# Jun-CEN/Open-World-Semantic-Segmentation

Measured on AMD Instinct MI355X. Metric: images/sec train-step, DeepLabV3+R101 768x768 bs=16; % HBM & MFMA roofline, higher is better.
Workload: dtype f16x2

## Files before the change

open-world-semantic-segmentation_amd/csrc/conv_choice.h:

```cpp
#pragma once
#include <cstdint>

#include "../../include/dmlnet_hip.h"

namespace conv_choice {

constexpr int CUS = 256;
constexpr int BK = 32;
constexpr int NTHREADS = 256;
constexpr int WS_MT = 9;
constexpr int WS_STAT_ROWS = 48;
constexpr int WS_NLD = 3;
constexpr int WB_THREADS = 512;
constexpr int WGW_TN = 128, WGW_TK = 256, WGW_NLD = 3;
constexpr int WG_MAX_JOBS = 12;

struct ConvSwitches {
    bool v1;
    int bm256, ws;
};

static inline int mul32(const int a, const int b) { return (int)((uint32_t)a * (uint32_t)b); }
static inline uintptr_t addr(const void* p) { return reinterpret_cast<uintptr_t>(p); }

static inline int64_t operand_bytes(const int B, const int Hi, const int Wi, const int ld, const int C, const int es) {
    return (((int64_t)mul32(B, Hi) * Wi - 1) * ld + C) * es;
}
static inline int blocks_for(const int64_t work_items, const int block, const int max_blocks = 256 * 8) {
    int64_t g = (work_items + block - 1) / block;
    if (g < 1) g = 1;
    if (g > max_blocks) g = max_blocks;
    return (int)g;
}

enum ConvFamily {
    CONV_REG = 0,
    CONV_RING,
    CONV_WS,
    CONV_X3
};

struct ConvChoice {
    int family;
    int elem_bytes;
    int mode;
    int bn, aligned;
    int bm, tmw, wpe;
    int mw, nw, pl, mt, epi;
    int nblk_m, nblk_n, tail_full, tail_q, nt_out;
    uint32_t x_bytes, w_bytes;
    uint32_t kx_bytes, kw_bytes;
    int grid, block;
    int stat_rows;
};

static inline int conv_m(const DmlConvDesc& d) { return mul32(mul32(d.B, d.Ho), d.Wo); }
static inline int conv_ktot(const DmlConvDesc& d) { return mul32(mul32(d.R, d.S), d.C); }
static inline int conv_f32_split(const DmlConvDesc& d) { return d.dtype == DML_F32 ? d.f32_split : 0; }
static inline bool conv_has_planes(const DmlConvDesc& d) { return conv_f32_split(d) == 2 && d.x_planes && d.w_planes; }
static inline bool conv_has_tail(const DmlConvDesc& d) { return d.tail_ws && d.tail_counters && d.tail_ws_elems > 0 && d.tail_counters_len > 0; }
static inline int conv_pad_x(const DmlConvDesc& d) { return d.pad_w_set ? d.pad_w : d.pad; }

static inline int64_t conv_x_bytes(const DmlConvDesc& d, const int es) { return operand_bytes(d.B, d.Hi, d.Wi, d.ldx, d.C, es); }
static inline int64_t conv_w_bytes(const DmlConvDesc& d, const int es) { return (int64_t)d.N * conv_ktot(d) * es; }

static inline bool conv_dma_eligible(const DmlConvDesc& d, const ConvSwitches& sw, const int64_t xb, const int64_t wb) {
    return !sw.v1 && (d.C % BK) == 0 && d.R * d.S <= 32 && d.N > 32 && xb < (1ll << 31) && wb < (1ll << 31);
}

static inline bool conv_ws_eligible(const DmlConvDesc& d, const ConvSwitches& sw, const int64_t xb, const int64_t wb) {
    if ((!sw.ws && d.ws_min_tiles <= 0) || !d.w_tiled || (d.C % BK) != 0 || d.R * d.S > 32 || (d.N % 128) != 0) return false;
    if (xb >= (1ll << 31) || wb >= (1ll << 31)) return false;
    if (d.ws_min_tiles <= 0 && d.R * d.S * d.C < 1024) return false;
    const int bn = (d.N % 256) == 0 ? 256 : 128, bm = (d.N % 256) == 0 ? 144 : 288;
    const int64_t ntiles = ((int64_t)conv_m(d) + bm - 1) / bm * (d.N / bn);
    return ntiles >= (d.ws_min_tiles > 0 ? d.ws_min_tiles : 192);
}
static inline bool ws_planes_short(const DmlConvDesc& d, const int mode) {
    return mode == 0 && (d.N % 256) == 0 && ((conv_m(d) + 143) / 144) * (d.N / 256) * 2 <= 256;
}
static inline int ws_planes_stat_rows(const DmlConvDesc& d, const int mode) {
    if (mode != 0) return 48;
    return (d.N == 64 || ws_planes_short(d, mode)) ? 48 : 144;
}
static inline bool conv_ws_planes_eligible(const DmlConvDesc& d, const int mode) {
    if (mode == 0 && d.accum) return false;
    if (!conv_has_planes(d) || !d.x_unscale || !d.w_unscale) return false;
    if (d.x_plane_stride >= (1ll << 30) || d.w_plane_stride >= (1ll << 30)) return false;
    if ((d.C % BK) != 0 || d.R * d.S > 32 || (d.N % 64) != 0) return false;
    if (mode == 1 && conv_ktot(d) < 2 * BK) return false;
    const bool post = d.post_scale != nullptr;
    if ((d.ldy & 3) != 0 || (post && d.post_res != nullptr && (d.post_ldres & 3) != 0) ||
        ((addr(d.y) | addr(d.bias) | (post ? addr(d.post_res) | addr(d.post_scale) | addr(d.post_shift) | addr(d.post_mean) : 0)) & 15) != 0)
        return false;
    return conv_x_bytes(d, 2) + (uint32_t)(d.x_plane_stride * 2) < (1ll << 31) && conv_w_bytes(d, 2) + (uint32_t)(d.w_plane_stride * 2) < (1ll << 31);
}

static inline int tail_split(const DmlConvDesc& d, const int ntiles, const int tile_rows, const int max_full, int* full_out) {
// ... 99 lines not shown
    *c = ConvChoice{};
    c->stat_rows = DML_STAT_ROWS;
    if (!dp) return DML_EINVAL;
    const DmlConvDesc& d = *dp;
    const bool planes_ok = d.dtype == DML_F32 && conv_ws_planes_eligible(d, d.mode);
    bool ws_ok = false;
    if (d.dtype == DML_BF16) {
        const int64_t xb = conv_x_bytes(d, 2), wb = conv_w_bytes(d, 2);
        ws_ok = conv_dma_eligible(d, sw, xb, wb) && conv_ws_eligible(d, sw, xb, wb);
    }
    if (planes_ok) c->stat_rows = ws_planes_stat_rows(d, d.mode);
    else if (ws_ok) c->stat_rows = WS_STAT_ROWS;

    if (!d.x || !d.w || !d.y) return DML_EINVAL;
    if (d.dtype != DML_F32 && d.dtype != DML_BF16) return DML_EINVAL;
    const int vec = d.dtype == DML_BF16 ? 8 : 4;
    if (d.C % vec || d.ldx % vec) return DML_EALIGN;
    if (d.mode != 0 && d.mode != 1) return DML_EINVAL;
    if (d.mode == 1 && d.stride != 1 && d.stride != 2) return DML_EUNSUPPORTED;
    if (d.B <= 0 || d.Ho <= 0 || d.Wo <= 0 || d.N <= 0 || d.R <= 0 || d.S <= 0) return DML_EINVAL;
    if ((int64_t)d.B * d.Ho * d.Wo >= (1ll << 31)) return DML_EINVAL;
    if (d.stats && d.bias) return DML_EINVAL;
    const int f32_split = conv_f32_split(d);
    if (f32_split < 0 || f32_split > 2) return DML_EINVAL;
    if (conv_has_planes(d)) {
        if (!d.x_unscale || !d.w_unscale || d.x_plane_stride <= 0 || d.w_plane_stride <= 0 ||
            d.x_plane_stride >= (1ll << 30) || d.w_plane_stride >= (1ll << 30))
            return DML_EINVAL;
        if ((addr(d.x_planes) & 15) || (addr(d.w_planes) & 15) || (d.x_plane_stride & 7) || (d.w_plane_stride & 7)) return DML_EALIGN;
    }
    if (d.w_tiled && (d.dtype != DML_BF16 || d.C % BK || d.N % 64)) return DML_EUNSUPPORTED;
    if (d.acc32) {
        if (d.mode != 1 || d.dtype != DML_BF16 || d.y_f32 || d.accum || d.res_dz || d.bnr_partials) return DML_EINVAL;
        if (d.N % 8 || d.ldy % 8 || d.acc32_ld % 4 || (addr(d.y) & 15) || (addr(d.acc32) & 15) || d.N <= 32) return DML_EALIGN;
    }
    if (d.res_dz) {
        if (d.mode != 1 || d.y_f32 || d.accum || !d.res_mask) return DML_EINVAL;
        if (d.dtype == DML_BF16) {
            if (d.N % 8 || d.ldy % 8 || d.res_ld % 8 || (addr(d.y) & 15) || (addr(d.res_dz) & 15) || d.N <= 32) return DML_EALIGN;
            if ((d.N & 63) == 0 && (addr(d.res_mask) & 7)) return DML_EALIGN;
        } else if (d.N % 64 || d.res_ld % 4 || ((addr(d.res_dz) | addr(d.res_mask)) & 15)) {
            return DML_EALIGN;
        }
    }
    if (conv_has_tail(d) && (addr(d.tail_ws) & 15)) return DML_EALIGN;
    if (d.post_scale) {
        if (d.mode != 0 || !d.post_shift || !d.post_mean || d.stats || d.bias || d.accum || d.y_f32) return DML_EINVAL;
        if (d.post_res && (d.post_ldres % vec || (addr(d.post_res) & 15))) return DML_EALIGN;
    }
    if (d.bnr_partials) {
        if (d.mode != 1 || d.y_f32 || !d.bnr_y || !d.bnr_mean || !d.bnr_invstd || (d.bnr_relu && !d.bnr_mask)) return DML_EINVAL;
        if (d.dtype == DML_BF16) {
            if (d.N % 8 || d.ldy % 8 || d.bnr_ldy % 8 || (addr(d.y) & 15) || (addr(d.bnr_y) & 15) || (addr(d.bnr_partials) & 15) || d.N <= 32)
                return DML_EUNSUPPORTED;
            if (d.bnr_relu && (d.N & 63) == 0 && (addr(d.bnr_mask) & 7)) return DML_EALIGN;
        } else {
            if (d.N % 64 || d.bnr_ldy % 4) return DML_EUNSUPPORTED;
            if (((addr(d.bnr_y) | addr(d.bnr_partials) | addr(d.bnr_mean) | addr(d.bnr_invstd) | (d.bnr_relu ? addr(d.bnr_mask) : 0)) & 15) != 0)
                return DML_EALIGN;
        }
    }
    if (d.bnr_partials && d.bnr_inc != 0 && (!d.accum || d.dtype != DML_F32 || d.res_dz)) return DML_EUNSUPPORTED;
    if (d.sub_grid) {
        if (d.mode != 1 || d.stride != 1 || d.dil != 1 || d.Hi != d.Ho || d.Wi != d.Wo || (unsigned)d.sub_y > 1u || (unsigned)d.sub_x > 1u ||
            d.dtype != DML_F32)
            return DML_EINVAL;
        if ((int64_t)4 * d.B * d.Ho * d.Wo * (int64_t)d.ldy * 4 >= (1ll << 31)) return DML_EUNSUPPORTED;
    }
    const bool own_geometry = d.sub_grid || conv_pad_x(d) != d.pad;
    if (own_geometry && (d.dtype == DML_BF16 || d.acc32)) return DML_EUNSUPPORTED;
    if (d.acc32) return conv_choose_kernel(d, sw, 2, 2, ws_ok, false, c);
    if (d.dtype == DML_BF16) return conv_choose_kernel(d, sw, 2, d.mode, ws_ok, false, c);
    if ((d.bnr_partials || d.res_dz || own_geometry) && !planes_ok) return DML_EUNSUPPORTED;
    if (d.f32_split == 2 && d.x_planes && d.x == d.x_planes && !planes_ok) return DML_EUNSUPPORTED;
    return conv_choose_kernel(d, sw, 4, d.mode, false, planes_ok, c);
}

enum WgradFamily {
    WGRAD_BIG = 0,
    WGRAD_WS,
    WGRAD_H2,
    WGRAD_N64,
    WGRAD_X3,
    WGRAD_PLAIN
};

struct ReduceLaunch {
    int grid_x, grid_y, block, splits, slab_stride, fold_only;
};

struct WgradChoice {
    int family;
    int lin;
    int elem_bytes;
    bool planes;
    bool use_ws;
    int tiles, cm;
    int nblk_n, nblk_k, splitk, slab_tiles;
    int grid, block;
    uint32_t x_bytes, dy_bytes;
    int nitems;
    int64_t nrs;
    int nreduce;
    ReduceLaunch reduce[2];
};

static inline int64_t wgrad_m(const DmlWgradDesc& d) { return (int64_t)d.B * d.Ho * d.Wo; }
static inline int wgrad_ktot(const DmlWgradDesc& d) { return mul32(mul32(d.R, d.S), d.C); }
static inline int64_t wgrad_x_bytes(const DmlWgradDesc& d, const int es) { return operand_bytes(d.B, d.Hi, d.Wi, d.ldx, d.C, es); }
static inline int64_t wgrad_dy_bytes(const DmlWgradDesc& d, const int es) { return ((wgrad_m(d) - 1) * d.ldy + d.N) * es; }

static inline bool wgrad_big_eligible(const DmlWgradDesc* d, const bool group) {
    if (!d) return false;
    const int64_t M = wgrad_m(*d), Ktot = (int64_t)d->R * d->S * d->C, tiles = (M + BK - 1) / BK;
    if (group) {
        if (!d->x || !d->dy || !d->dw) return false;
        if (d->C % 8 || d->ldx % 8 || d->N % 8 || d->ldy % 8) return false;
        if ((d->Cm > 0 ? d->Cm : d->C) > d->C) return false;
        if ((int64_t)d->N * Ktot < 65536) return false;
    }
    return d->dtype == DML_BF16 && d->N % 256 == 0 && (d->N / 256) * ((Ktot + 255) / 256) >= 4 && tiles >= 16 &&
           wgrad_x_bytes(*d, 2) < (1ll << 31) && wgrad_dy_bytes(*d, 2) < (1ll << 31) && (int64_t)(d->B + 1) * d->Hi * d->Wi < (1 << 24) &&
           M < (1 << 24) && d->ldx < (1 << 22) && d->ldy < (1 << 22);
}

template <class Score>
static inline int pick_splits(const int tiles, const int min_steps, const int64_t plane, const int64_t ws_elems, Score score) {
    int smax = tiles / min_steps;
    if (smax > 256) smax = 256;
    if ((int64_t)smax * plane > ws_elems) smax = (int)(ws_elems / plane);
    if (smax < 1) smax = 1;
    double best = -1e30;
    int sk = 1;
    for (int c = 1; c <= smax; ++c) {
        const int slab = (tiles + c - 1) / c;
        const int real = (tiles + slab - 1) / slab;
        const double s = score(slab, real);
        if (s > best + 1e-9) { best = s; sk = real; }
    }
    return sk;
}
static inline int flat_splits(const int base, const int tiles, const bool use_ws) {
    int splitk = use_ws ? (512 + base - 1) / base : (1024 + base - 1) / base;
    if (use_ws && tiles / 48 > splitk) splitk = tiles / 48;
    const int cap = (tiles + 7) / 8;
    if (splitk > cap) splitk = cap;
    if (splitk < 1) splitk = 1;
    return splitk;
}
static inline int finish_splits(int sk, const int tiles, const bool use_ws, const int64_t plane, const int64_t ws_elems, int* slab_tiles) {
    if (use_ws && (int64_t)sk * plane > ws_elems) sk = (int)(ws_elems / plane);
    if (use_ws && sk < 1) return 0;
    if (sk > tiles) sk = tiles > 0 ? tiles : 1;
    *slab_tiles = (tiles + sk - 1) / sk;
    return (tiles + *slab_tiles - 1) / *slab_tiles;
}

static inline int wgrad_choose(const DmlWgradDesc* dp, WgradChoice* c) {
    *c = WgradChoice{};
    if (!dp || !dp->x || !dp->dy || !dp->dw) return DML_EINVAL;
    const DmlWgradDesc& d = *dp;
    if (d.dtype != DML_F32 && d.dtype != DML_BF16) return DML_EINVAL;
    const int vec = d.dtype == DML_BF16 ? 8 : 4;
    if (d.C % vec || d.ldx % vec || d.N % vec || d.ldy % vec) return DML_EALIGN;
    if (wgrad_m(d) >= (1ll << 31)) return DML_EINVAL;
    const int M = (int)wgrad_m(d), Ktot = wgrad_ktot(d), N = d.N;
    if (d.dtype == DML_F32 && d.f32_split == 2 && d.x_planes && d.dy_planes) {
        if (!d.x_unscale || !d.dy_unscale || d.x_plane_stride <= 0 || d.dy_plane_stride <= 0) return DML_EINVAL;
        if ((addr(d.x_planes) & 15) || (addr(d.dy_planes) & 15) || (d.x_plane_stride & 7) || (d.dy_plane_stride & 7)) return DML_EALIGN;
        c->planes = d.C % 8 == 0 && d.N % 8 == 0 && d.ldx % 8 == 0 && d.ldy % 8 == 0 &&
                    wgrad_x_bytes(d, 2) + d.x_plane_stride * 2 < 0x7fffffffll && wgrad_dy_bytes(d, 2) + d.dy_plane_stride * 2 < 0x7fffffffll;
    }
    if (!c->planes && ((d.x_planes && d.x == d.x_planes) || (d.dy_planes && d.dy == d.dy_planes))) return DML_EUNSUPPORTED;
    const int tiles = c->tiles = (M + BK - 1) / BK;
    const int cm = c->cm = d.Cm > 0 ? d.Cm : d.C;
    if (cm > d.C) return DML_EINVAL;
    if (cm != d.C && !d.ws) return DML_EINVAL;
    const int64_t plane = (int64_t)N * Ktot;
    const bool use_ws = c->use_ws = d.ws != nullptr;
    c->lin = (d.R == 1 && d.S == 1 && d.stride == 1 && d.pad == 0) ? 1 : 0;
    c->nrs = (int64_t)N * d.R * d.S;
    c->block = NTHREADS;
    int sk = d.splitk, rblock = 256, rmax = 256 * 8;
    if (use_ws && wgrad_big_eligible(dp, false)) {
        c->family = WGRAD_BIG;
        c->nblk_n = N / 256;
        c->nblk_k = (Ktot + 255) / 256;
        const int base = c->nblk_n * c->nblk_k;
        if (sk <= 0)
            sk = pick_splits(tiles, 8, plane, d.ws_elems, [&](const int, const int real) {
                const int blocks = base * real;
                const int rnd = base < 6 ? 128 : 256;
                return (double)blocks / (double)(((blocks + rnd - 1) / rnd) * rnd);
            });
        c->block = WB_THREADS;
        c->x_bytes = (uint32_t)wgrad_x_bytes(d, 2);
        c->dy_bytes = (uint32_t)wgrad_dy_bytes(d, 2);
    } else if (c->planes && use_ws && N % WGW_TN == 0 && tiles >= 16 && (addr(d.ws) & 15) == 0) {
        c->family = WGRAD_WS;
        c->nblk_n = N / WGW_TN;
        c->nblk_k = (Ktot + WGW_TK - 1) / WGW_TK;
        const int base = c->nblk_n * c->nblk_k;
        if (sk <= 0)
            sk = pick_splits(tiles, 16, plane, d.ws_elems, [&](const int slab, const int real) {
                const int items = base * real;
                return -((double)((items + 255) / 256) * (slab * 1.45 + 8.0) + (double)real * (double)plane * 8.0 / 4.0e6);
            });
        c->block = (4 + WGW_NLD) * 64;
        c->x_bytes = (uint32_t)wgrad_x_bytes(d, 2);
        c->dy_bytes = (uint32_t)wgrad_dy_bytes(d, 2);
        rblock = 64;
        rmax = 256 * 8 * (256 / rblock);
    } else {
        const bool n64 = d.dtype == DML_BF16 && N <= 64 && d.R * d.S > 1;
        c->nblk_n = n64 ? 1 : (N + 127) / 128;
        c->nblk_k = n64 ? (Ktot + 255) / 256 : (Ktot + 127) / 128;
        if (sk <= 0) sk = flat_splits(c->nblk_n * c->nblk_k, tiles, use_ws);
        const int64_t x3_xb = wgrad_x_bytes(d, 4), x3_yb = wgrad_dy_bytes(d, 4);
        if (c->planes) {
            c->family = WGRAD_H2;
            c->x_bytes = (uint32_t)wgrad_x_bytes(d, 2);
            c->dy_bytes = (uint32_t)wgrad_dy_bytes(d, 2);
        } else if (n64) {
            c->family = WGRAD_N64;
        } else if (d.dtype == DML_F32 && d.f32_split && x3_xb < (int64_t)0x7fffffff && x3_yb < (int64_t)0x7fffffff) {
            c->family = WGRAD_X3;
            c->x_bytes = (uint32_t)x3_xb;
            c->dy_bytes = (uint32_t)x3_yb;
        } else {
            c->family = WGRAD_PLAIN;
            c->elem_bytes = d.dtype == DML_BF16 ? 2 : 4;
        }
    }
    sk = c->splitk = finish_splits(sk, tiles, use_ws, plane, d.ws_elems, &c->slab_tiles);
    if (sk < 1) return DML_EINVAL;
    c->grid = c->nblk_n * c->nblk_k * sk;
    if (c->family == WGRAD_WS) {
        c->nitems = c->grid;
        c->grid = c->nitems < 256 ? c->nitems : 256;
    }
    if (use_ws) {
        const int gx = blocks_for(c->nrs * cm, rblock, rmax);
        const int ychunks = (c->family != WGRAD_BIG && c->family != WGRAD_WS && c->nrs * cm < 65536 && sk > 64) ? (sk + 15) / 16 : 1;
        if (ychunks > 1) {
            c->nreduce = 2;
            c->reduce[0] = ReduceLaunch{gx, ychunks, rblock, sk, 1, 1};
            c->reduce[1] = ReduceLaunch{gx, 1, rblock, ychunks, 16, 0};
        } else {
            c->nreduce = 1;
            c->reduce[0] = ReduceLaunch{gx, 1, rblock, sk, 1, 0};
        }
    }
    return 0;
}

struct WgradGroupChoice {
    int n;
    int nblk_n[WG_MAX_JOBS], nblk_k[WG_MAX_JOBS], splitk[WG_MAX_JOBS], slab_tiles[WG_MAX_JOBS], cm[WG_MAX_JOBS];
    uint32_t x_bytes[WG_MAX_JOBS], dy_bytes[WG_MAX_JOBS];
    int64_t ws_off[WG_MAX_JOBS], nrs[WG_MAX_JOBS];
    int start[WG_MAX_JOBS + 1];
    int grid, block;
    int rgrid_x, rgrid_y, rblock;
};

static inline int wgrad_group_choose(const DmlWgradDesc* const* descs, const int n, const void* ws, const int64_t ws_elems, WgradGroupChoice* g) {
    *g = WgradGroupChoice{};
    if (!descs || n <= 0 || n > WG_MAX_JOBS || !ws) return DML_EINVAL;
    int base[WG_MAX_JOBS], tiles[WG_MAX_JOBS], sk[WG_MAX_JOBS];
    int64_t plane[WG_MAX_JOBS];
    double work = 0.0;
    int tbase = 0;
    for (int j = 0; j < n; ++j) {
        const DmlWgradDesc* d = descs[j];
        if (!wgrad_big_eligible(d, true)) return DML_EUNSUPPORTED;
        const int Ktot = wgrad_ktot(*d);
        g->nblk_n[j] = d->N / 256;
        g->nblk_k[j] = (Ktot + 255) / 256;
// ... 54 lines not shown
```

open-world-semantic-segmentation_amd/csrc/conv_device.h:

```cpp
#pragma once
#include "common.h"
#include "conv_choice.h"

namespace conv_device {

struct ConvArgs {
    const void* x;
    const void* w;
    void* y;
    const float* bias;
    float* stats;
    int B, Hi, Wi, C, ldx;
    int Ho, Wo, N, ldy;
    int R, S, stride, dil, pad;
    int M, Ktot;
    int y_f32, accum;
    int nblk_n, nblk_m;
    FastDiv div_wo, div_howo, div_c;
    float* unused0_;
    uint32_t x_bytes, w_bytes;
    int w_tiled;
    int ws_min_tiles;
    const void* x_planes;
    const void* w_planes;
    const float* x_unscale;
    const float* w_unscale;
    uint32_t x_plane_bytes, w_plane_bytes;
    const void* bnr_y;
    const uint8_t* bnr_mask;
    const float* bnr_mean;
    const float* bnr_invstd;
    float* bnr_partials;
    float* bnr_gmax;
    int bnr_ldy, bnr_relu;
    const float* post_scale;
    const float* post_shift;
    const float* post_mean;
    const void* post_res;
    int post_ldres, post_relu;
    float* tail_ws;
    int* tail_cnt;
    int tail_full, tail_q;
    int64_t tail_ws_elems_;
    int tail_cnt_len_;
    const void* res_dz;
    const uint8_t* res_mask;
    int res_ld;
    const float* acc32;
    int acc32_ld;
    int f32_split;
    int nt_out;
    int unused1_;
    int pad_x;
    int sub_grid, sub_y, sub_x;
    int bnr_inc;
};

__attribute__((visibility("hidden"))) void launch_conv_ws(const conv_choice::ConvChoice& c, const ConvArgs& a, hipStream_t st);
__attribute__((visibility("hidden"))) void launch_conv_ws_dgrad_planes(const conv_choice::ConvChoice& c, const ConvArgs& a, hipStream_t st);

}

namespace {

using namespace conv_device;
namespace cc = conv_choice;

constexpr int BK = 32;
constexpr int NTHREADS = 256;
constexpr int WS_MT = 9;
constexpr int WS_STAT_ROWS = 48;
constexpr int WS_NST = 6, WS_D = 2;
constexpr int WS_PLANES_NLD = 3;

typedef __bf16 mfma_bf16x8 __attribute__((ext_vector_type(8)));
typedef _Float16 mfma_f16x8 __attribute__((ext_vector_type(8)));
typedef unsigned int u32x4_ws __attribute__((ext_vector_type(4)));
typedef __attribute__((address_space(3))) void* lds_ptr_t;
template <int N> __device__ __forceinline__ void wait_vmcnt() { asm volatile("s_waitcnt vmcnt(%0)" ::"n"(N) : "memory"); }

__device__ __forceinline__ uint32_t ws_out_row(const ConvArgs& a, const uint32_t m) {
    if (!a.sub_grid) return m;
    if (m >= (uint32_t)a.M) return 4u * (uint32_t)a.M;
    const uint32_t b = fdiv(m, a.div_howo);
    const uint32_t rem = m - b * (uint32_t)(a.Ho * a.Wo);
    const uint32_t y2 = fdiv(rem, a.div_wo);
    const uint32_t x2 = rem - y2 * (uint32_t)a.Wo;
    return ((b * 2u * (uint32_t)a.Ho + 2u * y2 + (uint32_t)a.sub_y) * 2u * (uint32_t)a.Wo) + 2u * x2 + (uint32_t)a.sub_x;
}
__device__ __forceinline__ uint32_t ws_out_rows(const ConvArgs& a) { return a.sub_grid ? 4u * (uint32_t)a.M : (uint32_t)a.M; }

constexpr int WGRAD_DEPTH = 2;

__device__ __forceinline__ int xcd_remap(int bid, int nwg) {
    const int q = nwg >> 3, r = nwg & 7, xcd = bid & 7, slot = bid >> 3;
    const int base = xcd < r ? xcd * (q + 1) : r * (q + 1) + (xcd - r) * q;
    return base + slot;
}

template <typename T> __device__ __forceinline__ int swz_chunk(int row, int chunk);
template <> __device__ __forceinline__ int swz_chunk<bf16_t>(int row, int chunk) {
    return chunk ^ ((0x78 >> (((row >> 2) & 3) * 2)) & 3);
}
template <> __device__ __forceinline__ int swz_chunk<float>(int row, int chunk) { return chunk ^ (row & 7); }

template <int NT> __device__ __forceinline__ int frag_chan(int i, int g) {
    return NT == 4 ? (i >> 1) * 32 + g * 8 + (i & 1) * 4 : g * (4 * NT) + i * 4;
}
template <int NT> __device__ __forceinline__ int b_row(int i, int rho) { return frag_chan<NT>(i, rho >> 2) + (rho & 3); }
template <int NT> __device__ __forceinline__ int b_rho(int row) {
    return NT == 4 ? ((row >> 3) & 3) * 4 + (row & 3) : ((row / (4 * NT)) & 3) * 4 + (row & 3);
}

template <int CTRL> __device__ __forceinline__ float dpp_mov(float v) {
    return __int_as_float(__builtin_amdgcn_update_dpp(0, __float_as_int(v), CTRL, 0xF, 0xF, true));
}
__device__ __forceinline__ float row16_sum(float v) {
    v += dpp_mov<0xB1>(v);
    v += dpp_mov<0x4E>(v);
    v += dpp_mov<0x141>(v);
    v += dpp_mov<0x140>(v);
    return v;
}

typedef unsigned int u32x4_st __attribute__((ext_vector_type(4)));
typedef float f32x4_st __attribute__((ext_vector_type(4)));
__device__ __forceinline__ void st16(void* p, uint32_t a, uint32_t b, uint32_t c, uint32_t d, const bool nt) {
    const u32x4_st v = {a, b, c, d};
    if (nt) asm volatile("global_store_dwordx4 %0, %1, off nt" ::"v"(p), "v"(v) : "memory");
    else *reinterpret_cast<u32x4_st*>(p) = v;
}
__device__ __forceinline__ void st16f(float* p, float a, float b, float c, float d, const bool nt) {
    const f32x4_st v = {a, b, c, d};
    if (nt) asm volatile("global_store_dwordx4 %0, %1, off nt" ::"v"(p), "v"(v) : "memory");
    else *reinterpret_cast<f32x4_st*>(p) = v;
}

template <typename T, int NT, int MT, int MODE, bool WIDE_MASK = true, bool STATS_ONLY = false>
__device__ __forceinline__ void conv_epilogue(f32x4 (&acc)[NT][MT], const ConvArgs& a, const int mw0, const int nw0,
                                              const int lr, const int lq) {
    constexpr int TM = MT * 16;
    constexpr int CL = NT * 4;
    auto ch = [&](int c) { return nw0 + frag_chan<NT>(c >> 2, lq) + (c & 3); };

    if (a.stats != nullptr) {
        const int cnt = min(TM, max(0, a.M - mw0));
        if (cnt > 0) {
            const float inv = 1.0f / (float)cnt;
            const int grp = mw0 / TM;
            float* sg = a.stats + (int64_t)grp * a.N * 2;
            const bool pair_ok = (a.N & 1) == 0;
            const bool gather = pair_ok && nw0 + NT * 16 <= a.N;
            float S[NT][4], Q[NT][4];
#pragma unroll
            for (int i = 0; i < NT; ++i) {
                float s[4] = {0.f, 0.f, 0.f, 0.f};
#pragma unroll
                for (int j = 0; j < MT; ++j) {
                    const bool v = (mw0 + j * 16 + lr) < a.M;
#pragma unroll
                    for (int q = 0; q < 4; ++q) s[q] += v ? acc[i][j][q] : 0.f;
                }
#pragma unroll
                for (int q = 0; q < 4; ++q) s[q] = row16_sum(s[q]);
                float m2[4] = {0.f, 0.f, 0.f, 0.f};
#pragma unroll
                for (int j = 0; j < MT; ++j) {
                    const bool v = (mw0 + j * 16 + lr) < a.M;
#pragma unroll
                    for (int q = 0; q < 4; ++q) {
                        const float dlt = acc[i][j][q] - s[q] * inv;
                        m2[q] += v ? dlt * dlt : 0.f;
                    }
// ... 284 lines not shown
```

open-world-semantic-segmentation_amd/csrc/conv_igemm.hip:

```cpp
#include "conv_device.h"
#include <cstdlib>

namespace {

template <typename T, int BN, bool ALIGNED, int MODE>
__global__ __launch_bounds__(NTHREADS) __attribute__((amdgpu_waves_per_eu(3))) void conv_igemm_kernel(const ConvArgs a) {
    constexpr int BM = 128;
    constexpr int VEC = Elem<T>::VEC;
    constexpr int KV = BK / VEC;
    constexpr int RPP = NTHREADS / KV;
    constexpr int A_LD = BM / RPP;
    constexpr int B_LD = (BN + RPP - 1) / RPP;
    constexpr int TM = 64, TN = BN / 2;
    constexpr int MT = TM / 16, NT = TN / 16;

    __shared__ __attribute__((aligned(256))) T smem[2 * (BM + BN) * BK];
    auto As = [&](int buf) -> T* { return smem + buf * (BM + BN) * BK; };
    auto Bs = [&](int buf) -> T* { return smem + buf * (BM + BN) * BK + BM * BK; };

    const int tid = threadIdx.x, lane = tid & 63, wave = tid >> 6;
    const int wm = wave >> 1, wn = wave & 1;
    const int tile = xcd_remap(blockIdx.x, gridDim.x);
    const int blk_m = tile / a.nblk_n, blk_n = tile - blk_m * a.nblk_n;
    const int m0 = blk_m * BM, n0 = blk_n * BN;
// ... 548 lines not shown
        if (LA > 2 && kt + 2 < KT) wait_vmcnt<(LA > 2 ? 2 : 0) * NI>();
        else if (LA > 1 && kt + 1 < KT) wait_vmcnt<(LA > 1 ? 1 : 0) * NI>();
        else wait_vmcnt<0>();
        __builtin_amdgcn_s_barrier();
        if (kt + LA < KT) issue(kbeg + kt + LA, (kt + LA) % NST);
        const T* as = smem + (kt % NST) * STAGE + (wm * TM) * BK;
        const T* bs = smem + (kt % NST) * STAGE + BM * BK + (wn * TN) * BK;
        mfma_bf16x8 bf[NT], af[MT];
#pragma unroll
        for (int i = 0; i < NT; ++i)
            bf[i] = *reinterpret_cast<const mfma_bf16x8*>(bs + b_row<NT>(i, lr) * BK + swz_chunk<T>(lr, lq) * 8);
#pragma unroll
        for (int j = 0; j < MT; ++j) {
            const int row = j * 16 + lr;
            af[j] = *reinterpret_cast<const mfma_bf16x8*>(as + row * BK + swz_chunk<T>(row, lq) * 8);
        }
#pragma unroll
        for (int i = 0; i < NT; ++i)
#pragma unroll
            for (int j = 0; j < MT; ++j)
                acc[i][j] = __builtin_amdgcn_mfma_f32_16x16x32_bf16(bf[i], af[j], acc[i][j], 0, 0, 0);
    }
#pragma unroll
    for (int i = 0; i < NT; ++i)
#pragma unroll
        for (int j = 0; j < MT; ++j) asm volatile("" : "+v"(acc[i][j]));
    if (kparts > 1) {
        const int rt = tile - a.tail_full;
        typedef unsigned int u32x4_t __attribute__((ext_vector_type(4)));
        const __amdgpu_buffer_rsrc_t rs_ws = __builtin_amdgcn_make_buffer_rsrc(
            a.tail_ws + (int64_t)rt * kparts * (BM * BN), 0, kparts * BM * BN * 4, 0x00020000);
#pragma unroll
        for (int i = 0; i < NT; ++i)
#pragma unroll
            for (int j = 0; j < MT; ++j)
                __builtin_amdgcn_raw_buffer_store_b128(__builtin_bit_cast(u32x4_t, acc[i][j]), rs_ws,
                                                       (kpart * BM * BN + ((i * MT + j) * NTH + tid) * 4) * 4, 0, 16);
        asm volatile("s_waitcnt vmcnt(0)" ::: "memory");
        __syncthreads();
        int* flag = reinterpret_cast<int*>(smem);
        if (tid == 0) {
            const int ticket = __hip_atomic_fetch_add(a.tail_cnt + rt, 1, __ATOMIC_RELAXED, __HIP_MEMORY_SCOPE_AGENT);
            if (ticket == kparts - 1)
                __hip_atomic_store(a.tail_cnt + rt, 0, __ATOMIC_RELAXED, __HIP_MEMORY_SCOPE_AGENT);
            *flag = ticket;
        }
        __syncthreads();
        if (*flag != kparts - 1) return;
#pragma unroll
        for (int i = 0; i < NT; ++i)
#pragma unroll
            for (int j = 0; j < MT; ++j) acc[i][j] = (f32x4){0.f, 0.f, 0.f, 0.f};
        for (int p = 0; p < kparts; ++p) {
#pragma unroll
            for (int i = 0; i < NT; ++i)
#pragma unroll
                for (int j = 0; j < MT; ++j) {
                    const u32x4_t v = __builtin_amdgcn_raw_buffer_load_b128(
                        rs_ws, (p * BM * BN + ((i * MT + j) * NTH + tid) * 4) * 4, 0, 16);
                    acc[i][j] += __builtin_bit_cast(f32x4, v);
                }
        }
    }
    if constexpr (MT == 4) {
        conv_epilogue<T, NT, MT, MODE>(acc, a, m0 + wm * TM, n0 + wn * TN, lr, lq);
    } else {
#pragma unroll
        for (int h = 0; h < MT / 4; ++h) {
            f32x4 sub[NT][4];
#pragma unroll
            for (int i = 0; i < NT; ++i)
#pragma unroll
                for (int j = 0; j < 4; ++j) sub[i][j] = acc[i][h * 4 + j];
            conv_epilogue<T, NT, 4, MODE, false>(sub, a, m0 + wm * TM + h * 64, n0 + wn * TN, lr, lq);
        }
    }
}

static const conv_choice::ConvSwitches& conv_switches() {
    static const conv_choice::ConvSwitches s = {getenv("DML_CONV_V1") != nullptr, getenv("DML_CONV_BM256") ? atoi(getenv("DML_CONV_BM256")) : 1,
                                                getenv("DML_CONV_WS") ? atoi(getenv("DML_CONV_WS")) : 0};
    return s;
}

struct WgradArgs {
    const void* x;
    const void* dy;
    float* dw;
    int B, Hi, Wi, C, ldx;
    int Ho, Wo, N, ldy;
    int R, S, stride, dil, pad;
    int M, Ktot;
    int nblk_n, nblk_k;
    int slab_tiles;
    float* ws;
    FastDiv div_wo, div_howo, div_c;
    const void* x_planes;
    const void* dy_planes;
    const float* x_unscale;
    const float* dy_unscale;
    uint32_t x_plane_bytes, dy_plane_bytes;
};

template <typename T> struct WgLds;
template <> struct WgLds<float> { static constexpr int PITCH = 128 + 16; };
template <> struct WgLds<bf16_t> { static constexpr int PITCH = 128 + 8; };

__device__ __forceinline__ bf16x4 lds_tr16_b64(const bf16_t* p) {
    typedef short v4i16 __attribute__((ext_vector_type(4)));
    return __builtin_amdgcn_ds_read_tr16_b64_v4i16((v4i16 __attribute__((address_space(3)))*)(p));
}

template <typename T>
__global__ __launch_bounds__(NTHREADS) void conv_wgrad_kernel(const WgradArgs a) {
    constexpr int TILE = 128;
    constexpr int VEC = Elem<T>::VEC;
    constexpr int CV = TILE / VEC;
    constexpr int RPP = NTHREADS / CV;
    constexpr int LD = BK / RPP;
    constexpr int PITCH = WgLds<T>::PITCH;
    constexpr int MT = 4, NT = 4;

    __shared__ __attribute__((aligned(16))) T smem[2 * 2 * BK * PITCH];
    auto Ys = [&](int buf) -> T* { return smem + buf * 2 * BK * PITCH; };
    auto Xs = [&](int buf) -> T* { return smem + buf * 2 * BK * PITCH + BK * PITCH; };

    const int tid = threadIdx.x, lane = tid & 63, wave = tid >> 6;
    const int wn = wave >> 1, wk = wave & 1;
    const int ntile = a.nblk_n * a.nblk_k;
    const int logical = xcd_remap(blockIdx.x, gridDim.x);
    const int split = logical / ntile, tile_id = logical - split * ntile;
    const int blk_n = tile_id % a.nblk_n, blk_k = tile_id / a.nblk_n;
    const int n0 = blk_n * TILE, kc0 = blk_k * TILE;

    const T* __restrict__ X = static_cast<const T*>(a.x);
    const T* __restrict__ DY = static_cast<const T*>(a.dy);

    const int vcol = tid % CV, prow = tid / CV;
    const int kc = kc0 + vcol * VEC;
    const bool kc_ok = kc < a.Ktot;
    const uint32_t tap = fdiv((uint32_t)(kc_ok ? kc : 0), a.div_c);
    const int xc = (kc_ok ? kc : 0) - (int)tap * a.C;
    const int tr = (int)tap / a.S, ts = (int)tap - tr * a.S;
    const int dyo = tr * a.dil - a.pad, dxo = ts * a.dil - a.pad;
    const int yn = n0 + vcol * VEC;
    const bool yn_ok = yn < a.N;

    const int tile_beg = split * a.slab_tiles;
    const int tiles_total = (a.M + BK - 1) / BK;
    const int tile_end = min(tiles_total, tile_beg + a.slab_tiles);

    const bool lin1x1 = a.R == 1 && a.S == 1 && a.stride == 1 && a.pad == 0;
    uint4 y_reg[LD], x_reg[LD];
    auto load_tiles = [&](int t) {
#pragma unroll
        for (int j = 0; j < LD; ++j) {
            const int m = t * BK + prow + j * RPP;
            uint4 yv = make_uint4(0, 0, 0, 0), xv = make_uint4(0, 0, 0, 0);
            if (m < a.M) {
                if (yn_ok) yv = *reinterpret_cast<const uint4*>(DY + (int64_t)m * a.ldy + yn);
                if (kc_ok && lin1x1) {
                    xv = *reinterpret_cast<const uint4*>(X + (int64_t)m * a.ldx + xc);
                } else if (kc_ok) {
                    const uint32_t b = fdiv((uint32_t)m, a.div_howo);
                    const uint32_t rem = (uint32_t)m - b * (uint32_t)(a.Ho * a.Wo);
                    const uint32_t yo = fdiv(rem, a.div_wo);
                    const uint32_t xo = rem - yo * (uint32_t)a.Wo;
                    const int ys = (int)yo * a.stride + dyo, xs = (int)xo * a.stride + dxo;
                    if ((unsigned)ys < (unsigned)a.Hi && (unsigned)xs < (unsigned)a.Wi)
                        xv = *reinterpret_cast<const uint4*>(
                            X + ((int64_t)((int)b * a.Hi + ys) * a.Wi + xs) * a.ldx + xc);
                }
            }
            y_reg[j] = yv;
            x_reg[j] = xv;
        }
    };
    auto store_tiles = [&](int buf) {
#pragma unroll
        for (int j = 0; j < LD; ++j) {
            const int row = prow + j * RPP;
            int off;
            if constexpr (sizeof(T) == 2) {
                const int prow_ = (row & 0x13) | (((row >> 3) & 1) << 2) | (((row >> 2) & 1) << 3);
                off = (vcol >> 1) * 528 + prow_ * 16 + (vcol & 1) * 8;
            } else {
                off = row * PITCH + vcol * VEC;
            }
            *reinterpret_cast<uint4*>(Ys(buf) + off) = y_reg[j];
            *reinterpret_cast<uint4*>(Xs(buf) + off) = x_reg[j];
        }
    };

    f32x4 acc[NT][MT];
// ... 1053 lines not shown

template <typename T, int MODE>
void launch_conv(const cc::ConvChoice& c, const ConvArgs& a, hipStream_t st) {
    const dim3 grid(c.grid), block(c.block);
    switch (c.family) {
    case cc::CONV_RING:
        if constexpr (sizeof(T) == 2) {
            if (c.bm == 256)
                hipLaunchKernelGGL((conv_igemm_dma_kernel<128, MODE, 3, 2, 256, 128>), grid, block, 0, st, a, c.kx_bytes, c.kw_bytes);
            else if (c.bn == 128)
                hipLaunchKernelGGL((conv_igemm_dma_kernel<128, MODE, 3>), grid, block, 0, st, a, c.kx_bytes, c.kw_bytes);
            else
                hipLaunchKernelGGL((conv_igemm_dma_kernel<64, MODE, 3>), grid, block, 0, st, a, c.kx_bytes, c.kw_bytes);
        }
        break;
    case cc::CONV_X3:
        if constexpr (sizeof(T) == 4 && MODE != 2) {
            if (c.bn == 128) hipLaunchKernelGGL((conv_igemm_x3_kernel<128, MODE>), grid, block, 0, st, a);
            else hipLaunchKernelGGL((conv_igemm_x3_kernel<64, MODE>), grid, block, 0, st, a);
        }
        break;
    default:
        if constexpr (MODE != 2) {
            if (c.aligned) {
                if (c.bn == 128) hipLaunchKernelGGL((conv_igemm_kernel<T, 128, true, MODE>), grid, block, 0, st, a);
                else if (c.bn == 64) hipLaunchKernelGGL((conv_igemm_kernel<T, 64, true, MODE>), grid, block, 0, st, a);
                else hipLaunchKernelGGL((conv_igemm_kernel<T, 32, true, MODE>), grid, block, 0, st, a);
            } else {
                if (c.bn == 128) hipLaunchKernelGGL((conv_igemm_kernel<T, 128, false, MODE>), grid, block, 0, st, a);
                else if (c.bn == 64) hipLaunchKernelGGL((conv_igemm_kernel<T, 64, false, MODE>), grid, block, 0, st, a);
                else hipLaunchKernelGGL((conv_igemm_kernel<T, 32, false, MODE>), grid, block, 0, st, a);
            }
        }
        break;
    }
}

static void fill_wgrad_args(WgradArgs& a, const DmlWgradDesc* d, const bool planes) {
    a.x = d->x; a.dy = d->dy; a.dw = d->dw;
    a.B = d->B; a.Hi = d->Hi; a.Wi = d->Wi; a.C = d->C; a.ldx = d->ldx;
    a.Ho = d->Ho; a.Wo = d->Wo; a.N = d->N; a.ldy = d->ldy;
    a.R = d->R; a.S = d->S; a.stride = d->stride; a.dil = d->dil; a.pad = d->pad;
    a.M = d->B * d->Ho * d->Wo;
    a.Ktot = d->R * d->S * d->C;
    a.div_wo = make_fastdiv((uint32_t)d->Wo);
    a.div_howo = make_fastdiv((uint32_t)(d->Ho * d->Wo));
    a.div_c = make_fastdiv((uint32_t)d->C);
    a.x_planes = planes ? d->x_planes : nullptr; a.dy_planes = planes ? d->dy_planes : nullptr;
    a.x_unscale = planes ? d->x_unscale : nullptr; a.dy_unscale = planes ? d->dy_unscale : nullptr;
    a.x_plane_bytes = planes ? (uint32_t)(d->x_plane_stride * 2) : 0u;
    a.dy_plane_bytes = planes ? (uint32_t)(d->dy_plane_stride * 2) : 0u;
}

}

extern "C" int dml_conv_stat_rows(const DmlConvDesc* d) {
    cc::ConvChoice c;
    cc::conv_choose(d, conv_switches(), &c);
    return c.stat_rows;
}

extern "C" int dml_conv_igemm(const DmlConvDesc* d, void* stream) {
    cc::ConvChoice c;
    const int rc = cc::conv_choose(d, conv_switches(), &c);
    if (rc) return rc;
    const ConvArgs a = conv_args(d, c);
    hipStream_t st = static_cast<hipStream_t>(stream);
    if (c.family == cc::CONV_WS) {
        launch_conv_ws(c, a, st);
    } else if (c.elem_bytes == 2) {
        if (c.mode == 2) launch_conv<bf16_t, 2>(c, a, st);
        else if (c.mode == 1) launch_conv<bf16_t, 1>(c, a, st);
        else launch_conv<bf16_t, 0>(c, a, st);
    } else {
        if (c.mode == 1) launch_conv<float, 1>(c, a, st);
        else launch_conv<float, 0>(c, a, st);
    }
    DML_LAUNCH_CHECK();
    return 0;
}

extern "C" int dml_conv_wgrad(const DmlWgradDesc* d, void* stream) {
    cc::WgradChoice c;
    const int rc = cc::wgrad_choose(d, &c);
    if (rc) return rc;
    WgradArgs a;
    fill_wgrad_args(a, d, c.planes);
    a.nblk_n = c.nblk_n; a.nblk_k = c.nblk_k; a.slab_tiles = c.slab_tiles;
    a.ws = c.use_ws ? d->ws : nullptr;
    hipStream_t st = static_cast<hipStream_t>(stream);
    const dim3 grid(c.grid), block(c.block);
    switch (c.family) {
    case cc::WGRAD_BIG:
        hipLaunchKernelGGL(conv_wgrad_big_kernel<WGRAD_DEPTH>, grid, block, 0, st, a, c.x_bytes, c.dy_bytes);
        break;
    case cc::WGRAD_WS:
        if (c.lin) hipLaunchKernelGGL(conv_wgrad_ws_kernel<true>, grid, block, 0, st, a, c.x_bytes, c.dy_bytes, c.nitems);
        else hipLaunchKernelGGL(conv_wgrad_ws_kernel<false>, grid, block, 0, st, a, c.x_bytes, c.dy_bytes, c.nitems);
        break;
    case cc::WGRAD_H2:
        if (c.lin) hipLaunchKernelGGL(conv_wgrad_h2_kernel<true>, grid, block, 0, st, a, c.x_bytes, c.dy_bytes);
        else hipLaunchKernelGGL(conv_wgrad_h2_kernel<false>, grid, block, 0, st, a, c.x_bytes, c.dy_bytes);
        break;
    case cc::WGRAD_N64:
        hipLaunchKernelGGL(conv_wgrad_n64_kernel, grid, block, 0, st, a);
        break;
    case cc::WGRAD_X3:
        if (c.lin) hipLaunchKernelGGL(conv_wgrad_x3_kernel<true>, grid, block, 0, st, a, c.x_bytes, c.dy_bytes);
        else hipLaunchKernelGGL(conv_wgrad_x3_kernel<false>, grid, block, 0, st, a, c.x_bytes, c.dy_bytes);
        break;
    default:
        if (c.elem_bytes == 2) hipLaunchKernelGGL(conv_wgrad_kernel<bf16_t>, grid, block, 0, st, a);
        else hipLaunchKernelGGL(conv_wgrad_kernel<float>, grid, block, 0, st, a);
        break;
    }
    for (int i = 0; i < c.nreduce; ++i) {
        const cc::ReduceLaunch& r = c.reduce[i];
        hipLaunchKernelGGL(wgrad_reduce_kernel, dim3(r.grid_x, r.grid_y), dim3(r.block), 0, st, d->ws, d->dw, r.splits, c.nrs, c.cm, d->C,
                           r.slab_stride, r.fold_only);
    }
    DML_LAUNCH_CHECK();
    return 0;
}

extern "C" int dml_conv_wgrad_group_eligible(const DmlWgradDesc* d) { return cc::wgrad_big_eligible(d, true) ? 1 : 0; }

extern "C" int dml_conv_wgrad_group(const DmlWgradDesc* const* descs, int n, float* ws, int64_t ws_elems, void* stream) {
    cc::WgradGroupChoice c;
    const int rc = cc::wgrad_group_choose(descs, n, ws, ws_elems, &c);
    if (rc) return rc;
    WgradGroup g;
    ReduceGroup r;
    g.njobs = r.njobs = n;
    g.start[0] = 0;
    for (int j = 0; j < n; ++j) {
        const DmlWgradDesc* d = descs[j];
        WgradArgs& a = g.job[j];
        fill_wgrad_args(a, d, false);
        a.nblk_n = c.nblk_n[j]; a.nblk_k = c.nblk_k[j]; a.slab_tiles = c.slab_tiles[j];
        a.ws = ws + c.ws_off[j];
        g.xb[j] = c.x_bytes[j]; g.yb[j] = c.dy_bytes[j];
        g.start[j + 1] = c.start[j + 1];
        r.ws[j] = a.ws; r.dw[j] = d->dw; r.splits[j] = c.splitk[j]; r.Cm[j] = c.cm[j]; r.Cp[j] = d->C;
        r.NRS[j] = c.nrs[j];
    }
    hipStream_t st = static_cast<hipStream_t>(stream);
    hipLaunchKernelGGL(conv_wgrad_group_kernel<WGRAD_DEPTH>, dim3(c.grid), dim3(c.block), 0, st, g);
    hipLaunchKernelGGL(wgrad_reduce_group_kernel, dim3(c.rgrid_x, c.rgrid_y), dim3(c.rblock), 0, st, r);
    DML_LAUNCH_CHECK();
    return 0;
}
```

Baseline: 213.4.

## Add tap-reuse wgrad kernel for 64-channel 3x3 stride-1 convolutions

Adds a dedicated weight-gradient kernel for 3x3, pad-1, stride-1 convolutions with 64 input and output channels. It loads one input patch per row tile into LDS and reuses it for all nine taps, with a 3-stage async DMA pipeline over split f16 planes. The kernel computes hi/lo cross products with MFMA and writes split-K partials to the workspace for the existing reduce. It is on by default through an env switch and only applies to that narrow shape, so its effect on the whole train step depends on how many such layers DeepLabV3+ R101 has.

```diff
diff --git a/open-world-semantic-segmentation_amd/csrc/conv_choice.h b/open-world-semantic-segmentation_amd/csrc/conv_choice.h
--- a/open-world-semantic-segmentation_amd/csrc/conv_choice.h
+++ b/open-world-semantic-segmentation_amd/csrc/conv_choice.h
@@ -14,6 +14,8 @@
 constexpr int WB_THREADS = 512;
 constexpr int WGW_TN = 128, WGW_TK = 256, WGW_NLD = 3;
 constexpr int WG_MAX_JOBS = 12;
+constexpr int WGT_CH = 64;
+constexpr int WGT_MIN_STEPS = 8;
 
 struct ConvSwitches {
     bool v1;
@@ -279,7 +281,12 @@
     WGRAD_H2,
     WGRAD_N64,
     WGRAD_X3,
-    WGRAD_PLAIN
+    WGRAD_PLAIN,
+    WGRAD_TAP
+};
+
+struct WgradSwitches {
+    bool tap = false;
 };
 
 struct ReduceLaunch {
@@ -353,7 +360,12 @@
     return (tiles + *slab_tiles - 1) / *slab_tiles;
 }
 
-static inline int wgrad_choose(const DmlWgradDesc* dp, WgradChoice* c) {
+static inline bool wgrad_tap_eligible(const DmlWgradDesc& d, const bool planes, const bool use_ws) {
+    return planes && use_ws && (addr(d.ws) & 15) == 0 && d.R == 3 && d.S == 3 && d.stride == 1 && d.dil == 1 && d.pad == 1 &&
+           d.Hi == d.Ho && d.Wi == d.Wo && d.N == WGT_CH && d.C == WGT_CH && d.Wo % BK == 0;
+}
+
+static inline int wgrad_choose(const DmlWgradDesc* dp, WgradChoice* c, const WgradSwitches& sw = WgradSwitches{}) {
     *c = WgradChoice{};
     if (!dp || !dp->x || !dp->dy || !dp->dw) return DML_EINVAL;
     const DmlWgradDesc& d = *dp;
@@ -391,6 +403,14 @@
                 return (double)blocks / (double)(((blocks + rnd - 1) / rnd) * rnd);
             });
         c->block = WB_THREADS;
+        c->x_bytes = (uint32_t)wgrad_x_bytes(d, 2);
+        c->dy_bytes = (uint32_t)wgrad_dy_bytes(d, 2);
+    } else if (sw.tap && wgrad_tap_eligible(d, c->planes, use_ws)) {
+        c->family = WGRAD_TAP;
+        c->nblk_n = c->nblk_k = 1;
+        if (sk <= 0)
+            sk = pick_splits(tiles, WGT_MIN_STEPS, plane, d.ws_elems, [&](const int, const int real) { return (double)real / (double)CUS; });
+        if (sk > CUS) sk = CUS;
         c->x_bytes = (uint32_t)wgrad_x_bytes(d, 2);
         c->dy_bytes = (uint32_t)wgrad_dy_bytes(d, 2);
     } else if (c->planes && use_ws && N % WGW_TN == 0 && tiles >= 16 && (addr(d.ws) & 15) == 0) {
diff --git a/open-world-semantic-segmentation_amd/csrc/conv_device.h b/open-world-semantic-segmentation_amd/csrc/conv_device.h
--- a/open-world-semantic-segmentation_amd/csrc/conv_device.h
+++ b/open-world-semantic-segmentation_amd/csrc/conv_device.h
@@ -56,8 +56,28 @@
     int bnr_inc;
 };
 
+struct WgradArgs {
+    const void* x;
+    const void* dy;
+    float* dw;
+    int B, Hi, Wi, C, ldx;
+    int Ho, Wo, N, ldy;
+    int R, S, stride, dil, pad;
+    int M, Ktot;
+    int nblk_n, nblk_k;
+    int slab_tiles;
+    float* ws;
+    FastDiv div_wo, div_howo, div_c;
+    const void* x_planes;
+    const void* dy_planes;
+    const float* x_unscale;
+    const float* dy_unscale;
+    uint32_t x_plane_bytes, dy_plane_bytes;
+};
+
 __attribute__((visibility("hidden"))) void launch_conv_ws(const conv_choice::ConvChoice& c, const ConvArgs& a, hipStream_t st);
 __attribute__((visibility("hidden"))) void launch_conv_ws_dgrad_planes(const conv_choice::ConvChoice& c, const ConvArgs& a, hipStream_t st);
+__attribute__((visibility("hidden"))) void launch_conv_wgrad_tap(const conv_choice::WgradChoice& c, const WgradArgs& a, hipStream_t st);
 
 }
 
@@ -89,6 +109,11 @@
     return ((b * 2u * (uint32_t)a.Ho + 2u * y2 + (uint32_t)a.sub_y) * 2u * (uint32_t)a.Wo) + 2u * x2 + (uint32_t)a.sub_x;
 }
 __device__ __forceinline__ uint32_t ws_out_rows(const ConvArgs& a) { return a.sub_grid ? 4u * (uint32_t)a.M : (uint32_t)a.M; }
+
+__device__ __forceinline__ bf16x4 lds_tr16_b64(const bf16_t* p) {
+    typedef short v4i16 __attribute__((ext_vector_type(4)));
+    return __builtin_amdgcn_ds_read_tr16_b64_v4i16((v4i16 __attribute__((address_space(3)))*)(p));
+}
 
 constexpr int WGRAD_DEPTH = 2;
 
diff --git a/open-world-semantic-segmentation_amd/csrc/conv_igemm.hip b/open-world-semantic-segmentation_amd/csrc/conv_igemm.hip
--- a/open-world-semantic-segmentation_amd/csrc/conv_igemm.hip
+++ b/open-world-semantic-segmentation_amd/csrc/conv_igemm.hip
@@ -654,34 +654,14 @@
                                                 getenv("DML_CONV_WS") ? atoi(getenv("DML_CONV_WS")) : 0};
     return s;
 }
-
-struct WgradArgs {
-    const void* x;
-    const void* dy;
-    float* dw;
-    int B, Hi, Wi, C, ldx;
-    int Ho, Wo, N, ldy;
-    int R, S, stride, dil, pad;
-    int M, Ktot;
-    int nblk_n, nblk_k;
-    int slab_tiles;
-    float* ws;
-    FastDiv div_wo, div_howo, div_c;
-    const void* x_planes;
-    const void* dy_planes;
-    const float* x_unscale;
-    const float* dy_unscale;
-    uint32_t x_plane_bytes, dy_plane_bytes;
-};
+static const conv_choice::WgradSwitches& wgrad_switches() {
+    static const conv_choice::WgradSwitches s = {getenv("DML_WGRAD_TAP") ? atoi(getenv("DML_WGRAD_TAP")) != 0 : true};
+    return s;
+}
 
 template <typename T> struct WgLds;
 template <> struct WgLds<float> { static constexpr int PITCH = 128 + 16; };
 template <> struct WgLds<bf16_t> { static constexpr int PITCH = 128 + 8; };
-
-__device__ __forceinline__ bf16x4 lds_tr16_b64(const bf16_t* p) {
-    typedef short v4i16 __attribute__((ext_vector_type(4)));
-    return __builtin_amdgcn_ds_read_tr16_b64_v4i16((v4i16 __attribute__((address_space(3)))*)(p));
-}
 
 template <typename T>
 __global__ __launch_bounds__(NTHREADS) void conv_wgrad_kernel(const WgradArgs a) {
@@ -1901,7 +1881,7 @@
 
 extern "C" int dml_conv_wgrad(const DmlWgradDesc* d, void* stream) {
     cc::WgradChoice c;
-    const int rc = cc::wgrad_choose(d, &c);
+    const int rc = cc::wgrad_choose(d, &c, wgrad_switches());
     if (rc) return rc;
     WgradArgs a;
     fill_wgrad_args(a, d, c.planes);
@@ -1924,6 +1904,9 @@
     case cc::WGRAD_N64:
         hipLaunchKernelGGL(conv_wgrad_n64_kernel, grid, block, 0, st, a);
         break;
+    case cc::WGRAD_TAP:
+        launch_conv_wgrad_tap(c, a, st);
+        break;
     case cc::WGRAD_X3:
         if (c.lin) hipLaunchKernelGGL(conv_wgrad_x3_kernel<true>, grid, block, 0, st, a, c.x_bytes, c.dy_bytes);
         else hipLaunchKernelGGL(conv_wgrad_x3_kernel<false>, grid, block, 0, st, a, c.x_bytes, c.dy_bytes);
diff --git a/open-world-semantic-segmentation_amd/csrc/conv_wgrad_tap.hip b/open-world-semantic-segmentation_amd/csrc/conv_wgrad_tap.hip
--- /dev/null
+++ b/open-world-semantic-segmentation_amd/csrc/conv_wgrad_tap.hip
@@ -0,0 +1,143 @@
+#include "conv_device.h"
+
+namespace {
+
+constexpr int WGT_NST = 3;
+constexpr int WGT_PITCH = 32;
+constexpr int WGT_ROWPX = BK + 2, WGT_SLOTS = 3 * WGT_ROWPX;
+constexpr int WGT_YSUB = BK * WGT_PITCH;
+constexpr int WGT_XSUB = 4 * 1024;
+constexpr int WGT_YPL = 4 * WGT_YSUB, WGT_XPL = 4 * WGT_XSUB;
+constexpr int WGT_SB = 2 * WGT_YPL + 2 * WGT_XPL;
+constexpr int WGT_NI = 10;
+constexpr int WGT_KF = 18;
+static_assert(cc::WGT_CH == 64 && cc::BK == BK && 2 * WGT_KF * 16 == 9 * cc::WGT_CH, "conv_choice.h describes this kernel");
+static_assert((2 * WGT_ROWPX + 2 + BK) <= WGT_SLOTS && WGT_SLOTS * WGT_PITCH <= WGT_XSUB, "every tap's window lies inside the patch");
+
+__device__ __forceinline__ mfma_f16x8 wgt_frag(const char* p) {
+    const bf16x4 lo = lds_tr16_b64(reinterpret_cast<const bf16_t*>(p));
+    const bf16x4 hi = lds_tr16_b64(reinterpret_cast<const bf16_t*>(p + 16 * WGT_PITCH));
+    const bf16x8 v = {lo[0], lo[1], lo[2], lo[3], hi[0], hi[1], hi[2], hi[3]};
+    return __builtin_bit_cast(mfma_f16x8, v);
+}
+
+__device__ __forceinline__ constexpr int wgt_x_off(const int f) {
+    return 2 * WGT_YPL + (f & 3) * WGT_XSUB + (((f >> 2) / 3) * WGT_ROWPX + ((f >> 2) % 3)) * WGT_PITCH;
+}
+
+template <int WK>
+__device__ __forceinline__ void wgt_body(const WgradArgs& a, const u32x4_ws rs_x, const u32x4_ws rs_y, char* smem,
+                                         const int wave, const int lane, const int split, const int tile_beg, const int KT) {
+    constexpr uint32_t OOB = 0x80000000u;
+    const int wn = wave >> 1;
+    const int lr = lane & 15, lq = lane >> 4;
+
+    const int vec_b = (wave * 2 + (lane & 1)) * 16;
+    int x_dy[4], x_dx[4], x_off[4];
+#pragma unroll
+    for (int q = 0; q < 4; ++q) {
+        const int slot = q * 32 + (lane >> 1);
+        const int row = slot / WGT_ROWPX, col = slot - row * WGT_ROWPX;
+        x_dy[q] = slot < WGT_SLOTS ? row - 1 : -(1 << 20);
+        x_dx[q] = col - 1;
+        x_off[q] = ((row - 1) * a.Wi + (col - 1)) * (a.ldx * 2) + vec_b;
+    }
+    const int y_off = (lane >> 1) * (a.ldy * 2) + vec_b;
+    const uint32_t lds0 = (uint32_t)(uintptr_t)smem;
+    auto issue = [&](const int kt) {
+        const uint32_t sb = lds0 + (uint32_t)((kt % WGT_NST) * WGT_SB);
+        const uint32_t m0 = (uint32_t)(tile_beg + kt) * BK;
+        const uint32_t b = fdiv(m0, a.div_howo);
+        const uint32_t rem = m0 - b * (uint32_t)(a.Ho * a.Wo);
+        const int yo = (int)fdiv(rem, a.div_wo);
+        const int xo = (int)rem - yo * a.Wo;
+        const int base = (((int)b * a.Hi + yo) * a.Wi + xo) * (a.ldx * 2);
+#pragma unroll
+        for (int q = 0; q < 4; ++q) {
+            const bool ok = (unsigned)(yo + x_dy[q]) < (unsigned)a.Hi && (unsigned)(xo + x_dx[q]) < (unsigned)a.Wi;
+            const uint32_t voff = ok ? (uint32_t)(base + x_off[q]) : OOB;
+            const uint32_t dst = sb + (uint32_t)(2 * WGT_YPL + wave * WGT_XSUB + q * 1024);
+            ws_dma16(rs_x, dst, voff, 0u);
+            ws_dma16(rs_x, dst + WGT_XPL, voff, a.x_plane_bytes);
+        }
+        const uint32_t yv = m0 * (uint32_t)(a.ldy * 2) + (uint32_t)y_off;
+        ws_dma16(rs_y, sb + (uint32_t)(wave * WGT_YSUB), yv, 0u);
+        ws_dma16(rs_y, sb + (uint32_t)(WGT_YPL + wave * WGT_YSUB), yv, a.dy_plane_bytes);
+    };
+
+    f32x4 acc[2][WGT_KF];
+#pragma unroll
+    for (int i = 0; i < 2; ++i)
+#pragma unroll
+        for (int j = 0; j < WGT_KF; ++j) acc[i][j] = (f32x4){0.f, 0.f, 0.f, 0.f};
+
+    if (KT > 0) issue(0);
+    if (KT > 1) issue(1);
+    const int lane_off = (4 * lq + (lr >> 2)) * WGT_PITCH + (lr & 3) * 8;
+    for (int kt = 0; kt < KT; ++kt) {
+        if (kt + 1 < KT) wait_vmcnt<WGT_NI>();
+        else wait_vmcnt<0>();
+        __builtin_amdgcn_s_barrier();
+        if (kt + 2 < KT) issue(kt + 2);
+        const char* sb = smem + (kt % WGT_NST) * WGT_SB + lane_off;
+        mfma_f16x8 yh[2], yl[2];
+#pragma unroll
+        for (int i = 0; i < 2; ++i) {
+            yh[i] = wgt_frag(sb + (wn * 2 + i) * WGT_YSUB);
+            yl[i] = wgt_frag(sb + WGT_YPL + (wn * 2 + i) * WGT_YSUB);
+        }
+#pragma unroll
+        for (int j = 0; j < WGT_KF; j += 2) {
+            mfma_f16x8 xh[2], xl[2];
+#pragma unroll
+            for (int jj = 0; jj < 2; ++jj) {
+                xh[jj] = wgt_frag(sb + wgt_x_off(WK * WGT_KF + j + jj));
+                xl[jj] = wgt_frag(sb + wgt_x_off(WK * WGT_KF + j + jj) + WGT_XPL);
+            }
+#pragma unroll
+            for (int jj = 0; jj < 2; ++jj)
+#pragma unroll
+                for (int i = 0; i < 2; ++i) acc[i][j + jj] = __builtin_amdgcn_mfma_f32_16x16x32_f16(xh[jj], yl[i], acc[i][j + jj], 0, 0, 0);
+#pragma unroll
+            for (int jj = 0; jj < 2; ++jj)
+#pragma unroll
+                for (int i = 0; i < 2; ++i) acc[i][j + jj] = __builtin_amdgcn_mfma_f32_16x16x32_f16(xl[jj], yh[i], acc[i][j + jj], 0, 0, 0);
+#pragma unroll
+            for (int jj = 0; jj < 2; ++jj)
+#pragma unroll
+                for (int i = 0; i < 2; ++i) acc[i][j + jj] = __builtin_amdgcn_mfma_f32_16x16x32_f16(xh[jj], yh[i], acc[i][j + jj], 0, 0, 0);
+        }
+        asm volatile("s_waitcnt lgkmcnt(0)" ::: "memory");
+    }
+#pragma unroll
+    for (int i = 0; i < 2; ++i)
+#pragma unroll
+        for (int j = 0; j < WGT_KF; ++j) asm volatile("" : "+v"(acc[i][j]));
+    const float un = a.x_unscale[0] * a.dy_unscale[0];
+#pragma unroll
+    for (int i = 0; i < 2; ++i) {
+        const int n = wn * 32 + i * 16 + lr;
+        float* wrow = a.ws + ((int64_t)split * a.N + n) * a.Ktot + WK * WGT_KF * 16 + lq * 4;
+#pragma unroll
+        for (int j = 0; j < WGT_KF; ++j) *reinterpret_cast<f32x4*>(wrow + j * 16) = acc[i][j] * un;
+    }
+}
+
+__global__ __launch_bounds__(NTHREADS) void conv_wgrad_tap_kernel(const WgradArgs a, const uint32_t x_bytes, const uint32_t dy_bytes) {
+    __shared__ __attribute__((aligned(1024))) char smem[WGT_NST * WGT_SB];
+    const int tid = threadIdx.x, lane = tid & 63;
+    const int wave = __builtin_amdgcn_readfirstlane(tid >> 6);
+    const int split = xcd_remap(blockIdx.x, gridDim.x);
+    const int tiles_total = a.M / BK;
+    const int tile_beg = split * a.slab_tiles;
+    const int KT = min(tiles_total, tile_beg + a.slab_tiles) - tile_beg;
+    const u32x4_ws rs_x = ws_make_rsrc(a.x_planes, x_bytes + a.x_plane_bytes), rs_y = ws_make_rsrc(a.dy_planes, dy_bytes + a.dy_plane_bytes);
+    if (wave & 1) wgt_body<1>(a, rs_x, rs_y, smem, wave, lane, split, tile_beg, KT);
+    else wgt_body<0>(a, rs_x, rs_y, smem, wave, lane, split, tile_beg, KT);
+}
+
+}
+
+void conv_device::launch_conv_wgrad_tap(const cc::WgradChoice& c, const WgradArgs& a, hipStream_t st) {
+    hipLaunchKernelGGL(conv_wgrad_tap_kernel, dim3(c.grid), dim3(c.block), 0, st, a, c.x_bytes, c.dy_bytes);
+}
```

Result: no change. 214.6 (median of 6 runs) (+0.6%).
